# sunshinnnn/DSMnet

Measured on AMD Instinct MI355X. Metric: stereo pairs/sec forward, PSMNet D=192 384×1280, at 1/2/4/8 MI355X, higher is better.
Workload: dtype f32

## Files before the change

dsmnet_amd/csrc/basicblock2d.hpp:

```cpp
#pragma once

#ifndef DSM_BB_OFF
#define DSM_BB_OFF 0
#endif

template <int PM, int C_>
struct BbCfg {
  static constexpr int NP = Prec<PM>::NP, NPW = Prec<PM>::NPW;
  static constexpr int C = C_, NCH = C / 16, NT = C / 32;
  static constexpr int MG = 8 / NT;
  static constexpr int TY = 8, BY = TY + 4, BX = 36;
  static constexpr int MY = TY + 2, MX = 34, NMID = MY * MX;
  static constexpr int NMT = (NMID + 31) / 32;
  static constexpr int NVOX = BY * BX;
  static constexpr int THREADS = 512;
  static constexpr int NPF = (NVOX * 4 + THREADS - 1) / THREADS;
  static constexpr int PITCH = 32 * NP + 16;
  static constexpr int XIMG = NPF * 128 * PITCH;
  static constexpr int TCH = NMT * 32 * PITCH;
  static constexpr int IMGS = XIMG > NCH * TCH ? XIMG : NCH * TCH;
  static constexpr int LDS = IMGS + 4 * C * 4 + 64;
  static constexpr int WGS = 2 * LDS <= 160 * 1024 ? 2 : 1;
  static_assert(LDS <= 160 * 1024, "LDS");
};

template <int PM, int C>
__global__ __launch_bounds__(512, (BbCfg<PM, C>::WGS)) void basicblock2d_kernel(BbParams p) {
  using Cf = BbCfg<PM, C>;
  using frag = typename Prec<PM>::frag;
  constexpr int NP = Cf::NP, NPW = Cf::NPW, NCH = Cf::NCH, NT = Cf::NT, TY = Cf::TY, BX = Cf::BX, MX = Cf::MX,
                NMID = Cf::NMID, NVOX = Cf::NVOX, NPF = Cf::NPF, PITCH = Cf::PITCH, TCH = Cf::TCH;
  constexpr int AHEAD = 3;
  extern __shared__ __attribute__((aligned(16))) unsigned char lds_raw[];
  unsigned char* const ximg = lds_raw;
  unsigned char* const timg = lds_raw;
  float* const aff = reinterpret_cast<float*>(lds_raw + Cf::IMGS);
  float* const red = aff + 4 * C;

  const int tid = threadIdx.x, lane = tid & 63, wave = tid >> 6;
  const int r = lane & 31, h = lane >> 5;
  constexpr int MG = Cf::MG;
  const int nw = wave / MG, mg = wave % MG;
  int id = blockIdx.x;
  if (id >= p.ntiles) return;
  const int tx0 = (id % p.ntx) * 32; id /= p.ntx;
  const int ty0 = (id % p.nty) * TY;
  const int b = id / p.nty;

  const int ex = dsm_amax_exponent(*p.x_amax), ew1 = dsm_amax_exponent(*p.w1_amax), ew2 = dsm_amax_exponent(*p.w2_amax);
  const float sx = __builtin_bit_cast(float, __builtin_amdgcn_readfirstlane(__builtin_bit_cast(int, dsm_pow2f(ex))));
  const float so1 = dsm_pow2f(-(ex + ew1));
  if (tid < 4 * C) {
    const int c = tid % C, which = tid / C;
    const float* src = which == 0 ? p.scale1 : which == 1 ? p.shift1 : which == 2 ? p.scale2 : p.shift2;
    float v = src ? src[c] : ((which & 1) ? 0.f : 1.f);
    if (which == 0) v *= so1;
    aff[tid] = v;
  }

  constexpr unsigned OOBV = 0x80000000u;
  unsigned voff[NPF];
#pragma unroll
  for (int k = 0; k < NPF; ++k) {
    const int e = tid + k * Cf::THREADS;
    const int v = e >> 2, q = e & 3;
    const int yy = v / BX, xx = v % BX;
    const int y = ty0 - 2 + yy, x = tx0 - 2 + xx;
    const bool ok = v < NVOX && (unsigned)y < (unsigned)p.H && (unsigned)x < (unsigned)p.W;
    voff[k] = ok ? (unsigned)(4l * ((((long)b * p.H + y) * p.W + x) * C + 4 * q)) : OOBV;
  }
  f32x4 pf[NCH][NPF];
  static_for<0, NCH>([&](auto cc) {
    constexpr int c = decltype(cc)::value;
    const __amdgpu_buffer_rsrc_t rs = make_rsrc(reinterpret_cast<const char*>(p.x) + c * 64, p.xbytes);
    static_for<0, NPF>([&](auto kc) {
      if ((DSM_BB_OFF & 4) && p.B != 12345) pf[c][decltype(kc)::value] = f32x4{1.f, 0.5f, 0.25f, 2.f};
      else pf[c][decltype(kc)::value] = buffer_load16(rs, voff[decltype(kc)::value], 0);
    });
  });
  const unsigned lane16 = lane * 16u;
  const int wr_off = (tid >> 2) * PITCH + (tid & 3) * 8;

  frag wq[AHEAD][NP];
  const unsigned wlane = lane16 + (unsigned)nw * (NPW * 64 * 16);
  auto wload = [&](const __amdgpu_buffer_rsrc_t& rs, auto ic, unsigned wb) {
    constexpr int item = decltype(ic)::value;
#pragma unroll
    for (int q = 0; q < NP; ++q)
      wq[item % AHEAD][q] = __builtin_bit_cast(
          frag, buffer_load16(rs, wlane, wb + (item * NT * NPW + q) * (64 * 16)));
  };
  constexpr unsigned WCH = 9 * NT * NPW * 64 * 16;

  constexpr int NM1 = (Cf::NMT + MG - 1) / MG;
  int xbase[NM1];
  bool mt_on[NM1];
#pragma unroll
  for (int m = 0; m < NM1; ++m) {
    const int mt = mg + MG * m;
    mt_on[m] = mt < Cf::NMT;
    const int v = min(32 * mt + r, NMID - 1);
    xbase[m] = ((v / MX) * BX + v % MX) * PITCH + h * 16;
  }
  f32x16 acc1[NM1];
#pragma unroll
  for (int m = 0; m < NM1; ++m)
#pragma unroll
    for (int i = 0; i < 16; ++i) acc1[m][i] = 0.f;
  const __amdgpu_buffer_rsrc_t w1rs = make_rsrc(p.w1, p.wbytes);
  static_for<0, AHEAD - 1>([&](auto ic) { wload(w1rs, ic, 0u); });
  static_for<0, NCH>([&](auto cc) {
    constexpr int c = decltype(cc)::value;
    if constexpr (c > 0) __syncthreads();
    static_for<0, NPF>([&](auto kc) {
      constexpr int k = decltype(kc)::value;
      unsigned lo[NP], hi[NP];
      split_pair<PM>(pf[c][k].x, pf[c][k].y, sx, lo);
      split_pair<PM>(pf[c][k].z, pf[c][k].w, sx, hi);
#pragma unroll
      for (int q = 0; q < NP; ++q) {
        u32x2 v; v.x = lo[q]; v.y = hi[q];
        *reinterpret_cast<u32x2*>(ximg + wr_off + k * (128 * PITCH) + q * 32) = v;
      }
    });
    __syncthreads();
    static_for<0, 9>([&](auto ic) {
      constexpr int item = decltype(ic)::value;
      constexpr int tap_off = ((item / 3) * BX + item % 3) * PITCH;
      if constexpr (item + AHEAD - 1 < 9) wload(w1rs, std::integral_constant<int, item + AHEAD - 1>{}, c * WCH);
      else if constexpr (c + 1 < NCH) wload(w1rs, std::integral_constant<int, item + AHEAD - 1 - 9>{}, (c + 1) * WCH);
      frag xq[NM1][NP];
#pragma unroll
      for (int m = 0; m < NM1; ++m)
        if (mt_on[m]) {
#pragma unroll
          for (int q = 0; q < NP; ++q)
            xq[m][q] = *reinterpret_cast<const frag*>(ximg + xbase[m] + tap_off + q * 32);
        }
      __builtin_amdgcn_sched_barrier(0);
#pragma unroll
      for (int m = 0; m < NM1; ++m)
        if (mt_on[m] && (!(DSM_BB_OFF & 1) || p.B == 12345)) mma32<PM>(acc1[m], wq[item % AHEAD], xq[m]);
      __builtin_amdgcn_sched_barrier(0);
    });
  });
  constexpr int R2 = 8 / MG;
  const int xo = tx0 + r;
  Residual rr[R2];
#pragma unroll
  for (int m = 0; m < R2; ++m) {
    const int yo = ty0 + R2 * mg + m;
    if (p.skip && xo < p.W && yo < p.H) load_residual(rr[m], p.x + (((long)b * p.H + yo) * p.W + xo) * C + 32 * nw + 4 * h);
  }
  const __amdgpu_buffer_rsrc_t w2rs = make_rsrc(p.w2, p.wbytes);
  static_for<0, AHEAD - 1>([&](auto ic) { wload(w2rs, ic, 0u); });

  float tmax = 0.f;
#pragma unroll
  for (int m = 0; m < NM1; ++m) {
    if (!mt_on[m]) continue;
    const int v = 32 * (mg + MG * m) + r;
    const int y = ty0 - 1 + v / MX, x = tx0 - 1 + v % MX;
    const bool inside = v < NMID && (unsigned)y < (unsigned)p.H && (unsigned)x < (unsigned)p.W;
#pragma unroll
    for (int g = 0; g < 4; ++g) {
      const int cb = 32 * nw + 8 * g + 4 * h;
      const f32x4 sc = *reinterpret_cast<const f32x4*>(aff + cb), sh = *reinterpret_cast<const f32x4*>(aff + C + cb);
#pragma unroll
      for (int i = 0; i < 4; ++i) {
        float t = fmaxf(acc1[m][4 * g + i] * sc[i] + sh[i], 0.f);
        t = inside ? t : 0.f;
        acc1[m][4 * g + i] = t;
        tmax = fmaxf(tmax, t);
      }
    }
  }
#pragma unroll
  for (int o = 32; o; o >>= 1) tmax = fmaxf(tmax, __shfl_xor(tmax, o));
  if (lane == 0) red[wave] = tmax;
  __syncthreads();
  tmax = fmaxf(fmaxf(fmaxf(red[0], red[1]), fmaxf(red[2], red[3])), fmaxf(fmaxf(red[4], red[5]), fmaxf(red[6], red[7])));
  const int et = dsm_amax_exponent(tmax);
  const float st = dsm_pow2f(et);
#pragma unroll
  for (int m = 0; m < NM1; ++m) {
    if (!mt_on[m] || ((DSM_BB_OFF & 16) && p.B != 12345)) continue;
    const int v = 32 * (mg + MG * m) + r;
#pragma unroll
    for (int g = 0; g < 4; ++g) {
      unsigned lo[NP], hi[NP];
      split_pair<PM>(acc1[m][4 * g], acc1[m][4 * g + 1], st, lo);
      split_pair<PM>(acc1[m][4 * g + 2], acc1[m][4 * g + 3], st, hi);
#pragma unroll
      for (int q = 0; q < NP; ++q) {
        u32x2 w; w.x = lo[q]; w.y = hi[q];
        *reinterpret_cast<u32x2*>(timg + (2 * nw + (g >> 1)) * TCH + v * PITCH + q * 32 + 16 * (g & 1) + 8 * h) = w;
      }
    }
  }
  __syncthreads();

  f32x16 acc2[R2];
#pragma unroll
  for (int m = 0; m < R2; ++m)
#pragma unroll
    for (int i = 0; i < 16; ++i) acc2[m][i] = 0.f;
  const int tbase = ((R2 * mg) * MX + r) * PITCH + h * 16;
  static_for<0, NCH>([&](auto cc) {
    constexpr int c = decltype(cc)::value;
    static_for<0, 9>([&](auto ic) {
      constexpr int item = decltype(ic)::value;
      constexpr int tap_off = ((item / 3) * MX + item % 3) * PITCH;
      if constexpr (item + AHEAD - 1 < 9) wload(w2rs, std::integral_constant<int, item + AHEAD - 1>{}, c * WCH);
      else if constexpr (c + 1 < NCH) wload(w2rs, std::integral_constant<int, item + AHEAD - 1 - 9>{}, (c + 1) * WCH);
      frag xq[R2][NP];
#pragma unroll
      for (int m = 0; m < R2; ++m)
#pragma unroll
        for (int q = 0; q < NP; ++q)
          xq[m][q] = *reinterpret_cast<const frag*>(timg + c * TCH + tbase + m * (MX * PITCH) + tap_off + q * 32);
      __builtin_amdgcn_sched_barrier(0);
#pragma unroll
      for (int m = 0; m < R2; ++m)
        if (!(DSM_BB_OFF & 2) || p.B == 12345) mma32<PM>(acc2[m], wq[item % AHEAD], xq[m]);
      __builtin_amdgcn_sched_barrier(0);
    });
  });

  float am = 0.f;
  if (xo < p.W && (!(DSM_BB_OFF & 8) || p.B == 12345)) {
    const float so2 = dsm_pow2f(-(et + ew2));
    Affine af;
#pragma unroll
    for (int g = 0; g < 4; ++g) {
      af.sc[g] = *reinterpret_cast<const f32x4*>(aff + 2 * C + 32 * nw + 8 * g + 4 * h) * so2;
      af.sh[g] = *reinterpret_cast<const f32x4*>(aff + 3 * C + 32 * nw + 8 * g + 4 * h);
    }
#pragma unroll
    for (int m = 0; m < R2; ++m) {
      const int yo = ty0 + R2 * mg + m;
      if (yo < p.H)
        store_tile<C>(acc2[m], af, p.relu, p.y + (((long)b * p.H + yo) * p.W + xo) * C + 32 * nw + 4 * h, rr[m], p.skip != 0, am);
    }
  }
  flush_amax8(p.y_amax, am, red + 8);
}

template <int PM, int C>
int launch_basicblock2d(BbParams p, hipStream_t s) {
  using Cf = BbCfg<PM, C>;
  p.ntx = dsm_cdiv(p.W, 32); p.nty = dsm_cdiv(p.H, Cf::TY);
  const long nt = (long)p.B * p.nty * p.ntx;
  if (nt >= (1L << 30)) return DSM_ERR_UNSUPPORTED;
  p.ntiles = (int)nt;
  static thread_local bool configured = false;
  if (!configured) {
    if (hipFuncSetAttribute((const void*)basicblock2d_kernel<PM, C>, hipFuncAttributeMaxDynamicSharedMemorySize, Cf::LDS) != hipSuccess)
      return DSM_ERR_LAUNCH;
    configured = true;
  }
  hipLaunchKernelGGL((basicblock2d_kernel<PM, C>), dim3((unsigned)nt), dim3(Cf::THREADS), Cf::LDS, s, p);
  return dsm_launch_status();
}
```

dsmnet_amd/csrc/build.py:

```python
import os
import subprocess
import sys
from concurrent.futures import ThreadPoolExecutor

HERE = os.path.dirname(os.path.abspath(__file__))
SOURCES = ["abi.hip", "corr1d.hip", "cost_volume.hip", "soft_argmin.hip", "conv3d.hip", "conv_f16.hip",
           "conv3d_bwd.hip", "bn3d.hip", "decoder.hip", "spp.hip", "warp.hip",
           "selfsup.hip", "color.hip", "sepvol.hip", "suploss.hip"]
LIB = os.path.join(HERE, "libdsmnet_hip.so")
HIPCC = os.environ.get("HIPCC", "/opt/rocm/bin/hipcc")
FLAGS = ["--offload-arch=gfx950", "-O3", "-std=c++17", "-fPIC",
         "-Wall", "-Wno-unused-function"] + os.environ.get("HIPCC_EXTRA", "").split()


def _stale(out, deps):
    if not os.path.exists(out):
        return True
    t = os.path.getmtime(out)
    return any(os.path.getmtime(d) > t for d in deps)


def build(force=False, verbose=True, stamps=False):
    if stamps:
        lib = os.path.join(HERE, "libdsmnet_hip_stamps.so")
        srcs = [os.path.join(HERE, s) for s in SOURCES]
        extra = ["-DDSM_ABLATE=%s" % os.environ["DSM_ABLATE"]] if os.environ.get("DSM_ABLATE") else []
        cmd = [HIPCC] + FLAGS + ["-DDSM_STAMPS"] + extra + ["-shared", "-o", lib] + srcs
        print(" ".join(cmd), flush=True)
        subprocess.run(cmd, check=True)
        return lib
    hdrs = [os.path.join(HERE, "common.hpp"), os.path.join(HERE, "conv_split.hpp"), os.path.join(HERE, "conv_zs.hpp"), os.path.join(HERE, "deconv_zs.hpp"), os.path.join(HERE, "conv_common.hpp"),
            os.path.join(HERE, "..", "..", "include", "dsmnet_hip.h")]
    srcs = [os.path.join(HERE, s) for s in SOURCES if os.path.exists(os.path.join(HERE, s))]
    objs = []
    jobs = []
    for s in srcs:
        o = s[:-4] + ".o"
        objs.append(o)
        if force or _stale(o, [s] + hdrs):
            jobs.append([HIPCC] + FLAGS + ["-c", s, "-o", o])

    def run(cmd):
        if verbose:
            print(" ".join(cmd), flush=True)
        r = subprocess.run(cmd, capture_output=True, text=True)
        if r.returncode != 0:
            raise RuntimeError("hipcc failed:\n%s\n%s" % (r.stdout, r.stderr))
        if verbose and r.stderr.strip():
            print(r.stderr)

    with ThreadPoolExecutor(max_workers=min(4, max(1, len(jobs)))) as ex:
        list(ex.map(run, jobs))
    if jobs or force or _stale(LIB, objs):
        run([HIPCC, "--offload-arch=gfx950", "-shared", "-fPIC", "-o", LIB] + objs)
    return LIB


if __name__ == "__main__":
    print(build(force="--force" in sys.argv, stamps="--stamps" in sys.argv))
```

Measured before the change: 215.3.

## Double-buffer input prefetch and LDS fragment loads in 2D basic block

Input channel-chunk prefetch now uses a two-slot ring, and the load for chunk c+2 is issued after chunk c is staged to LDS. Before, every chunk was loaded up front, so register use grew with the chunk count. Both conv stages also software-pipeline the LDS fragment reads, loading the next tap's fragments into a second buffer before the current tap's MMAs run. The second stage is flattened across channel chunks so the pipeline carries over chunk boundaries. The build script now tracks every .hpp header for staleness, so edits to basicblock2d.hpp trigger a rebuild. The cost is extra registers for the doubled xq buffers.

```diff
diff --git a/dsmnet_amd/csrc/basicblock2d.hpp b/dsmnet_amd/csrc/basicblock2d.hpp
--- a/dsmnet_amd/csrc/basicblock2d.hpp
+++ b/dsmnet_amd/csrc/basicblock2d.hpp
@@ -69,15 +69,16 @@
     const bool ok = v < NVOX && (unsigned)y < (unsigned)p.H && (unsigned)x < (unsigned)p.W;
     voff[k] = ok ? (unsigned)(4l * ((((long)b * p.H + y) * p.W + x) * C + 4 * q)) : OOBV;
   }
-  f32x4 pf[NCH][NPF];
-  static_for<0, NCH>([&](auto cc) {
+  f32x4 pf[2][NPF];
+  auto request = [&](auto cc) {
     constexpr int c = decltype(cc)::value;
     const __amdgpu_buffer_rsrc_t rs = make_rsrc(reinterpret_cast<const char*>(p.x) + c * 64, p.xbytes);
     static_for<0, NPF>([&](auto kc) {
-      if ((DSM_BB_OFF & 4) && p.B != 12345) pf[c][decltype(kc)::value] = f32x4{1.f, 0.5f, 0.25f, 2.f};
-      else pf[c][decltype(kc)::value] = buffer_load16(rs, voff[decltype(kc)::value], 0);
-    });
-  });
+      if ((DSM_BB_OFF & 4) && p.B != 12345) pf[c & 1][decltype(kc)::value] = f32x4{1.f, 0.5f, 0.25f, 2.f};
+      else pf[c & 1][decltype(kc)::value] = buffer_load16(rs, voff[decltype(kc)::value], 0);
+    });
+  };
+  request(std::integral_constant<int, 0>{});
   const unsigned lane16 = lane * 16u;
   const int wr_off = (tid >> 2) * PITCH + (tid & 3) * 8;
 
@@ -109,38 +110,45 @@
     for (int i = 0; i < 16; ++i) acc1[m][i] = 0.f;
   const __amdgpu_buffer_rsrc_t w1rs = make_rsrc(p.w1, p.wbytes);
   static_for<0, AHEAD - 1>([&](auto ic) { wload(w1rs, ic, 0u); });
+  request(std::integral_constant<int, 1>{});
   static_for<0, NCH>([&](auto cc) {
     constexpr int c = decltype(cc)::value;
     if constexpr (c > 0) __syncthreads();
     static_for<0, NPF>([&](auto kc) {
       constexpr int k = decltype(kc)::value;
       unsigned lo[NP], hi[NP];
-      split_pair<PM>(pf[c][k].x, pf[c][k].y, sx, lo);
-      split_pair<PM>(pf[c][k].z, pf[c][k].w, sx, hi);
+      split_pair<PM>(pf[c & 1][k].x, pf[c & 1][k].y, sx, lo);
+      split_pair<PM>(pf[c & 1][k].z, pf[c & 1][k].w, sx, hi);
 #pragma unroll
       for (int q = 0; q < NP; ++q) {
         u32x2 v; v.x = lo[q]; v.y = hi[q];
         *reinterpret_cast<u32x2*>(ximg + wr_off + k * (128 * PITCH) + q * 32) = v;
       }
     });
+    if constexpr (c + 2 < NCH) request(std::integral_constant<int, (c + 2 < NCH ? c + 2 : 0)>{});
     __syncthreads();
+    frag xq[2][NM1][NP];
+    auto xload = [&](auto ic) {
+      constexpr int item = decltype(ic)::value;
+      constexpr int tap_off = ((item / 3) * BX + item % 3) * PITCH;
+#pragma unroll
+      for (int m = 0; m < NM1; ++m)
+        if (mt_on[m]) {
+#pragma unroll
+          for (int q = 0; q < NP; ++q)
+            xq[item & 1][m][q] = *reinterpret_cast<const frag*>(ximg + xbase[m] + tap_off + q * 32);
+        }
+    };
+    xload(std::integral_constant<int, 0>{});
     static_for<0, 9>([&](auto ic) {
       constexpr int item = decltype(ic)::value;
-      constexpr int tap_off = ((item / 3) * BX + item % 3) * PITCH;
       if constexpr (item + AHEAD - 1 < 9) wload(w1rs, std::integral_constant<int, item + AHEAD - 1>{}, c * WCH);
       else if constexpr (c + 1 < NCH) wload(w1rs, std::integral_constant<int, item + AHEAD - 1 - 9>{}, (c + 1) * WCH);
-      frag xq[NM1][NP];
+      if constexpr (item + 1 < 9) xload(std::integral_constant<int, item + 1>{});
+      __builtin_amdgcn_sched_barrier(0);
 #pragma unroll
       for (int m = 0; m < NM1; ++m)
-        if (mt_on[m]) {
-#pragma unroll
-          for (int q = 0; q < NP; ++q)
-            xq[m][q] = *reinterpret_cast<const frag*>(ximg + xbase[m] + tap_off + q * 32);
-        }
-      __builtin_amdgcn_sched_barrier(0);
-#pragma unroll
-      for (int m = 0; m < NM1; ++m)
-        if (mt_on[m] && (!(DSM_BB_OFF & 1) || p.B == 12345)) mma32<PM>(acc1[m], wq[item % AHEAD], xq[m]);
+        if (mt_on[m] && (!(DSM_BB_OFF & 1) || p.B == 12345)) mma32<PM>(acc1[m], wq[item % AHEAD], xq[item & 1][m]);
       __builtin_amdgcn_sched_barrier(0);
     });
   });
@@ -206,26 +214,30 @@
 #pragma unroll
     for (int i = 0; i < 16; ++i) acc2[m][i] = 0.f;
   const int tbase = ((R2 * mg) * MX + r) * PITCH + h * 16;
-  static_for<0, NCH>([&](auto cc) {
-    constexpr int c = decltype(cc)::value;
-    static_for<0, 9>([&](auto ic) {
-      constexpr int item = decltype(ic)::value;
+  {
+    frag xq[2][R2][NP];
+    auto xload = [&](auto sc) {
+      constexpr int s = decltype(sc)::value, c = s / 9, item = s % 9;
       constexpr int tap_off = ((item / 3) * MX + item % 3) * PITCH;
+#pragma unroll
+      for (int m = 0; m < R2; ++m)
+#pragma unroll
+        for (int q = 0; q < NP; ++q)
+          xq[s & 1][m][q] = *reinterpret_cast<const frag*>(timg + c * TCH + tbase + m * (MX * PITCH) + tap_off + q * 32);
+    };
+    xload(std::integral_constant<int, 0>{});
+    static_for<0, 9 * NCH>([&](auto sc) {
+      constexpr int s = decltype(sc)::value, c = s / 9, item = s % 9;
       if constexpr (item + AHEAD - 1 < 9) wload(w2rs, std::integral_constant<int, item + AHEAD - 1>{}, c * WCH);
       else if constexpr (c + 1 < NCH) wload(w2rs, std::integral_constant<int, item + AHEAD - 1 - 9>{}, (c + 1) * WCH);
-      frag xq[R2][NP];
+      if constexpr (s + 1 < 9 * NCH) xload(std::integral_constant<int, s + 1>{});
+      __builtin_amdgcn_sched_barrier(0);
 #pragma unroll
       for (int m = 0; m < R2; ++m)
-#pragma unroll
-        for (int q = 0; q < NP; ++q)
-          xq[m][q] = *reinterpret_cast<const frag*>(timg + c * TCH + tbase + m * (MX * PITCH) + tap_off + q * 32);
-      __builtin_amdgcn_sched_barrier(0);
-#pragma unroll
-      for (int m = 0; m < R2; ++m)
-        if (!(DSM_BB_OFF & 2) || p.B == 12345) mma32<PM>(acc2[m], wq[item % AHEAD], xq[m]);
-      __builtin_amdgcn_sched_barrier(0);
-    });
-  });
+        if (!(DSM_BB_OFF & 2) || p.B == 12345) mma32<PM>(acc2[m], wq[item % AHEAD], xq[s & 1][m]);
+      __builtin_amdgcn_sched_barrier(0);
+    });
+  }
 
   float am = 0.f;
   if (xo < p.W && (!(DSM_BB_OFF & 8) || p.B == 12345)) {
diff --git a/dsmnet_amd/csrc/build.py b/dsmnet_amd/csrc/build.py
--- a/dsmnet_amd/csrc/build.py
+++ b/dsmnet_amd/csrc/build.py
@@ -29,8 +29,8 @@
         print(" ".join(cmd), flush=True)
         subprocess.run(cmd, check=True)
         return lib
-    hdrs = [os.path.join(HERE, "common.hpp"), os.path.join(HERE, "conv_split.hpp"), os.path.join(HERE, "conv_zs.hpp"), os.path.join(HERE, "deconv_zs.hpp"), os.path.join(HERE, "conv_common.hpp"),
-            os.path.join(HERE, "..", "..", "include", "dsmnet_hip.h")]
+    hdrs = sorted(os.path.join(HERE, h) for h in os.listdir(HERE) if h.endswith(".hpp"))
+    hdrs.append(os.path.join(HERE, "..", "..", "include", "dsmnet_hip.h"))
     srcs = [os.path.join(HERE, s) for s in SOURCES if os.path.exists(os.path.join(HERE, s))]
     objs = []
     jobs = []
```

Measured after the change: 215.7, median of 6. Within noise of the previous version (+0.2%).
